# ZechengLi19/CIM

Hardware: AMD Instinct MI355X
Metric: images/sec training step (ResNet-50 VOC, ~1k proposals/img) at 1/2/4/8 GPU (higher is better)
Workload: dtype fp32

## Files before the change

### cim_amd/_lib.py

```python
import ctypes
import os

from ctypes import c_float, c_int, c_longlong, c_void_p

HERE = os.path.dirname(os.path.abspath(__file__))
LIB_PATH = os.environ.get("CIM_HIP_LIB") or os.path.join(HERE, "libcim_hip.so")

_P = c_void_p
SIGNATURES = {
    "cim_roi_align_fwd": [_P, _P, _P] + [c_int] * 6 + [c_float, c_int, c_int, _P],
    "cim_roi_align_fwd_ws": [_P, _P, _P] + [c_int] * 6 + [c_float, c_int, c_int, _P, _P],
    "cim_roi_align_maskcat_fwd_ws": [_P, _P, _P, _P] + [c_int] * 6 + [c_float, c_int, c_int, _P, _P],
    "cim_roi_align_wino7_pair_fwd": [_P, _P, _P, _P, _P] + [c_int] * 7 + [c_float, c_int, c_int, _P, _P],
    "cim_roi_align_bwd_ws": [_P, _P, _P] + [c_int] * 6 + [c_float, c_int, c_int, _P, c_int, _P, _P],
    "cim_roi_align_maskcat_bwd_ws": [_P, _P, _P, _P] + [c_int] * 6 + [c_float, c_int, c_int, _P, c_int, _P, _P],
    "cim_roi_align_bwd_workspace": [c_int, c_int, c_int, c_int],
    "cim_roi_align_bwd_scratch": [c_int, c_int, c_int, c_int, c_int],
    "cim_roi_align_bwd": [_P, _P, _P] + [c_int] * 6 + [c_float, c_int, c_int, _P, _P],
    "cim_roi_align_maskcat_fwd": [_P, _P, _P, _P] + [c_int] * 6 + [c_float, c_int, c_int, _P],
    "cim_roi_align_maskcat_bwd": [_P, _P, _P, _P] + [c_int] * 6 + [c_float, c_int, c_int, _P, _P],
    "cim_roi_align_forms": [c_int] * 9 + [_P] * 3,
    "cim_maxpool2d_out_size": [c_int, c_int, c_int, c_int],
    "cim_maxpool2d_fwd": [_P, _P, _P, c_int, c_int, c_int, c_int, c_int, c_int, _P],
    "cim_maxpool2d_bwd": [_P, _P, _P, c_int, c_int, c_int, c_int, c_int, c_int, _P],
    "cim_upsample_nearest_fwd": [_P, _P, c_int, c_int, c_int, c_int, c_int, _P],
    "cim_upsample_nearest_bwd": [_P, _P, c_int, c_int, c_int, c_int, _P],
    "cim_image_prep": [_P, c_int, c_int, _P, c_int, c_int, c_longlong, c_int, ctypes.c_double, c_int, _P, _P],
    "cim_mask_pack": [_P, _P, c_int, c_int, _P],
    "cim_mask_iou_pair": [_P, c_int, c_int, _P, _P, _P, _P],
    "cim_asy_flag": [_P, c_int, c_float, _P, _P],
    "cim_asy_prep": [_P, c_int, _P, c_int, _P, _P, _P],
    "cim_mining_step": [_P, _P, _P],
    "cim_mining_lds_bytes": [c_int, c_int],
    "cim_mining_sync_bytes": [],
    "cim_gemm_small_splits": [c_int, c_int, c_int],
    "cim_gemm_small_f32": [_P, _P, _P] + [c_int] * 8 + [_P, _P, _P, _P, _P, c_float, _P, c_int, c_int, _P, _P],
    "cim_conv1x1_bwd_workspace": [c_int, c_int, c_int, c_int],
    "cim_conv1x1_bn_act_bwd": [_P] * 8 + [c_float, c_int] + [_P] * 5 + [c_int] * 4 + [_P, _P, _P, _P, _P, c_int] + [c_int, _P, _P, c_float] + [_P] * 4 + [c_int],
    "cim_bn_part_finish": [_P, c_int, _P],
    "cim_conv3x3_nchw_splits": [c_int] * 5,
    "cim_conv3x3_nchw_f32": [_P, _P, _P] + [c_int] * 6 + [_P, _P, _P, _P, _P, c_float, _P, c_int, c_int, _P, _P],
    "cim_conv7x7_nchw_f32": [_P, _P, _P] + [c_int] * 5 + [_P, _P, _P, _P, c_float, c_int, _P],
    "cim_conv3x3_nchw_bwd_workspace": [c_int] * 6,
    "cim_conv3x3_dx_parts": [c_int] * 3,
    "cim_conv3x3_nchw_bn_act_bwd": [_P] * 8 + [c_float, c_int] + [_P] * 5 + [c_int] * 7 + [_P, _P, _P, _P, _P, c_int] + [c_int, _P, _P, c_float] + [_P] * 4,
    "cim_conv3x3_wt_multi": [_P, c_int, _P],
    "cim_bn_act_fwd": [_P, _P, _P, _P, _P, _P, c_float, _P, c_int, c_int, c_int, c_int, _P],
    "cim_bn_act_bwd_chunks": [c_int, c_int, c_int],
    "cim_bn_act_bwd": [_P, _P, _P, _P, _P, _P, c_float, _P, _P, _P, _P, c_int, c_int, c_int, c_int, _P],
    "cim_sgd_multi": [_P, _P, c_int, c_float, c_int, _P],
    "cim_gemm_pair_splits": [c_int, c_int, c_int],
    "cim_gemm_pair": [_P, _P, _P, _P] + [c_int] * 6 + [c_int, c_int, c_int, c_int, _P, _P, _P, _P, c_int, c_int, c_int, _P],
    "cim_gemm_pair_batched": [_P, _P, _P] + [c_int] * 6 + [c_int, c_int, c_int, c_longlong, c_longlong, c_longlong,
                              _P, _P, c_int, c_int, c_int, _P],
    "cim_pair_scales": [_P, c_int, _P, _P, c_int, c_int, _P],
    "cim_pair_split": [_P, _P, c_int, c_int, c_int, c_int, c_int, c_int, c_longlong, c_longlong, _P, _P, _P],
    "cim_pair_amax": [_P, c_longlong, _P, _P],
    "cim_pair_masked_stats": [_P, _P, c_int, c_int, _P, _P, _P],
# ... 57 lines not shown
    lib.cim_last_error.restype = ctypes.c_char_p
    lib.cim_last_error.argtypes = []
    lib.cim_abi_version.restype = c_int
    if lib.cim_abi_version() != ABI_VERSION:
        raise CimHipError("%s exports ABI %d, this package binds ABI %d: rebuild with `python -m cim_amd.build`"
                          % (LIB_PATH, lib.cim_abi_version(), ABI_VERSION))
    for name, argtypes in SIGNATURES.items():
        fn = getattr(lib, name)
        fn.argtypes = argtypes
        fn.restype = c_longlong if name in ("cim_conv1x1_bwd_workspace", "cim_conv3x3_nchw_bwd_workspace", "cim_roi_align_bwd_workspace", "cim_roi_align_bwd_scratch", "cim_mining_lds_bytes", "cim_mining_sync_bytes", "cim_detect_ws_bytes") or name in _LONG_RETURNING else c_int
    _lib = lib
    return lib


_LONG_RETURNING = {"cim_segm_rle_decode_ws_bytes", "cim_segm_image_ws_bytes", "cim_segm_record_bytes", "cim_segm_accumulate_ws_bytes", "cim_prop_ws_bytes"}
VALUE_RETURNING = _LONG_RETURNING | {"cim_segm_words"} | {"cim_maxpool2d_out_size", "cim_conv3x3_dx_parts", "cim_mining_sync_bytes", "cim_conv1x1_bwd_workspace", "cim_conv3x3_nchw_bwd_workspace", "cim_conv3x3_nchw_splits", "cim_gemm_small_splits", "cim_mining_lds_bytes", "cim_bn_act_bwd_chunks", "cim_gemm_pair_splits", "cim_roi_align_bwd_workspace", "cim_roi_align_bwd_scratch", "cim_detect_ws_bytes"}


PURE = {"cim_maxpool2d_out_size", "cim_conv3x3_dx_parts", "cim_gemm_small_splits", "cim_conv3x3_nchw_splits", "cim_conv1x1_bwd_workspace", "cim_conv3x3_nchw_bwd_workspace",
        "cim_bn_act_bwd_chunks", "cim_gemm_pair_splits"}
_PURE_VALUES = {}


def call(name, *args):
    if name in PURE:
        key = (name,) + args
        v = _PURE_VALUES.get(key)
        if v is None:
            v = _PURE_VALUES[key] = getattr(load(), name)(*args)
        return v
    lib = load()
    rc = getattr(lib, name)(*args)
    if name in VALUE_RETURNING:
        return rc
# ... 15 lines not shown
```

### cim_amd/csrc/conv1x1.hip

```cpp
#include "common.h"
#include "../../include/cim_hip.h"

#ifndef CIM_BODY_PRIO_LEVEL
#define CIM_BODY_PRIO_LEVEL 3
#endif
#if CIM_BODY_PRIO_LEVEL > 0
#define CIM_BODY_PRIO() __builtin_amdgcn_s_setprio(CIM_BODY_PRIO_LEVEL)
#else
#define CIM_BODY_PRIO()
#endif
namespace {

#ifndef CIM_SMALL_BK
#define CIM_SMALL_BK 32
#endif
#ifndef CIM_SMALL_ABL
#define CIM_SMALL_ABL 0
#endif
constexpr int SBM = 64, SBN = 64, SBK = CIM_SMALL_BK;
constexpr int SLD = 68;
typedef float f32x16 __attribute__((ext_vector_type(16)));
typedef float f32x4u __attribute__((ext_vector_type(4), aligned(4)));
__device__ __forceinline__ float4 ld4(const float* p) {
    const f32x4u v = *reinterpret_cast<const f32x4u*>(p);
    return make_float4(v.x, v.y, v.z, v.w);
}

struct SmallArgs {
    const float* A; const float* B; float* C; float* Xraw;
    const float* gamma; const float* beta; const float* mean; const float* var; const float* res;
    float eps;
    int M, N, K, lda, ldb, ldc;
    int a_mcontig, b_kcontig, relu, bn;
    int splits; float* ws;
    const float* colbias;
    const float* mask; const float* mgamma; const float* mvar; float meps;
    const float* mxr; const float* mmean; float* mpart; int mparts;
    int res_w, res_ws, res_hw;
};
struct InputBn { const float* y; const float* gamma; const float* var; float eps;
                 const float* xr; const float* mean; float* part; };

typedef unsigned int u32x4 __attribute__((ext_vector_type(4)));
typedef __amdgpu_buffer_rsrc_t rsrc_t;
__device__ __forceinline__ rsrc_t make_rsrc(const float* p, long long floats) {
    return __builtin_amdgcn_make_buffer_rsrc(const_cast<float*>(p), 0, (int)(unsigned)(floats * 4), 0x00020000);
}
__device__ __forceinline__ float4 bld4(rsrc_t r, unsigned byte_off) {
    const u32x4 v = __builtin_amdgcn_raw_buffer_load_b128(r, byte_off, 0, 0);
// ... 85 lines not shown
    __device__ __forceinline__ bool in(int c) const { return c < N; }
    __device__ __forceinline__ int col(int c) const { return c; }
    __device__ __forceinline__ int group(int c0) const { return c0 >> 5; }
};
struct ColParity {
    static constexpr bool splitk = false;
    int Wc, W, py, px, Nc, group0;
    __device__ __forceinline__ bool in(int c) const { return c < Nc; }
    __device__ __forceinline__ int col(int c) const {
        const int yc = c / Wc, xc = c - yc * Wc;
        return (2 * yc + py) * W + 2 * xc + px;
    }
    __device__ __forceinline__ int group(int c0) const { return group0 + (c0 >> 5); }
};
template <class Map>
__device__ __forceinline__ void small_epilogue(const SmallArgs& g, const f32x16& acc, int row0, int col0, int lane, int split, const Map& cm) {
#if CIM_SMALL_ABL == 2
    if (row0 + lane >= 0) return;
#endif
    const int nc = col0 + (lane & 31);
    if (Map::splitk && g.splits > 1) {
        if (cm.in(nc)) {
#pragma unroll
            for (int r = 0; r < 16; ++r) {
                const int row = row0 + 8 * (r >> 2) + 4 * (lane >> 5) + (r & 3);
                if (row < g.M) g.ws[((size_t)split * g.M + row) * g.N + cm.col(nc)] = acc[r];
            }
        }
        return;
    }
    const int col = cm.col(nc);
    if (g.mpart == nullptr) {
        if (cm.in(nc)) {
#pragma unroll
            for (int r = 0; r < 16; ++r) {
                const int row = row0 + 8 * (r >> 2) + 4 * (lane >> 5) + (r & 3);
                if (row < g.M) small_finish(g, row, col, acc[r]);
            }
        }
        return;
    }
#pragma unroll
    for (int r = 0; r < 16; ++r) {
        const int row = row0 + 8 * (r >> 2) + 4 * (lane >> 5) + (r & 3);
        float s1 = 0.0f, s2 = 0.0f;
        if (cm.in(nc) && row < g.M) small_finish(g, row, col, acc[r], s1, s2);
        small_put_part(g, row, cm.group(col0), lane, s1, s2);
    }
}


template <bool AM, bool BKc, int WN>
__global__ __launch_bounds__(128 * WN) void gemm_small_kernel(const SmallArgs g) {
    CIM_BODY_PRIO();
    constexpr int NT = 128 * WN, BNT = 32 * WN;
    constexpr int PA = SBM * 8 / NT, PB = BNT * 8 / NT;
    __shared__ __attribute__((aligned(16))) float As[2][SBK * SLD];
    __shared__ __attribute__((aligned(16))) float Bs[2][SBK * SLD];
    const int tid = threadIdx.x, lane = tid & 63, wave = tid >> 6;
    const int wm = wave / WN, wn = wave % WN;
    const int tiles_n = (g.N + BNT - 1) / BNT;
    const int tile = blockIdx.x;
    const int m0 = (tile / tiles_n) * SBM, n0 = (tile % tiles_n) * BNT;
    const int split = blockIdx.y;
    const int kper = ((g.K + g.splits - 1) / g.splits + SBK - 1) / SBK * SBK;
    const int kbeg = split * kper, kend = min(g.K, kbeg + kper);
#if CIM_SMALL_ABL == 4
    if (g.M > 0) return;
// ... 53 lines not shown
            SM_GLOAD(ra0, rb0, min(s + 2, last))
            SM_MMA(0)
            if (s + 1 < nslab) SM_PUT(ra1, rb1, 1, s + 1)
            __syncthreads();
            if (s + 1 >= nslab) break;
            SM_GLOAD(ra1, rb1, min(s + 3, last))
            SM_MMA(1)
            if (s + 2 < nslab) SM_PUT(ra0, rb0, 0, s + 2)
            __syncthreads();
        }
    }
#undef SM_GLOAD
#undef SM_PUT
#undef SM_MMA

    small_epilogue(g, acc, m0 + wm * 32, n0 + wn * 32, lane, split, ColIdentity{g.N});
}

__device__ __forceinline__ float splitk_sum(const float* __restrict__ ws, size_t i, size_t mn, int splits) {
    float v = ws[i];
    for (int k0 = 1; k0 < splits; k0 += 8) {
        float p[8];
#pragma unroll
        for (int j = 0; j < 8; ++j) p[j] = k0 + j < splits ? ws[(size_t)(k0 + j) * mn + i] : 0.0f;
#pragma unroll
        for (int j = 0; j < 8; ++j)
            if (k0 + j < splits) v += p[j];
    }
    return v;
}
__global__ __launch_bounds__(256) void small_splitk_reduce_kernel(const SmallArgs g) {
// ... 76 lines not shown
#pragma unroll
        for (int k = 0; k < 8; ++k) { a1 += sh[0][k][threadIdx.x]; a2 += sh[1][k][threadIdx.x]; }
        if (d.dbeta) d.dbeta[c] = a1;
        if (d.dgamma) d.dgamma[c] = a2 * rsqrtf(d.var[c] + d.eps);
    }
}

enum { CONV_FWD = 0, CONV_DX = 1, CONV_DW = 2 };
struct ConvGeom { int H, W, Ho, Wo, stride, cin, cout; float inv_w; int dil; };

#ifndef CIM_CONV3_BK
#define CIM_CONV3_BK 32
#endif
constexpr int CBK = CIM_CONV3_BK;
template <int MODE, int KS = 3>
__global__ __launch_bounds__(256) void conv3x3_small_kernel(const SmallArgs g, const ConvGeom c) {
    CIM_BODY_PRIO();
    constexpr int TAPS = KS * KS;
    constexpr int NT = 256, PA = SBM * (CBK / 4) / NT, PB = SBN * (CBK / 4) / NT;
    extern __shared__ __attribute__((aligned(16))) float c3_smem[];
    float (*As)[CBK * SLD] = reinterpret_cast<float (*)[CBK * SLD]>(c3_smem);
    float (*Bs)[CBK * SLD] = reinterpret_cast<float (*)[CBK * SLD]>(c3_smem + 2 * CBK * SLD);
    const int tid = threadIdx.x, lane = tid & 63, wave = tid >> 6;
    const int wm = wave >> 1, wn = wave & 1;
    const int tiles_n = (g.N + SBN - 1) / SBN;
    const int m0 = (blockIdx.x / tiles_n) * SBM, n0 = (blockIdx.x % tiles_n) * SBN;
    const int split = blockIdx.y;
    const int kper = ((g.K + g.splits - 1) / g.splits + CBK - 1) / CBK * CBK;
    const int kbeg = split * kper, kend = min(g.K, kbeg + kper);

    const rsrc_t RA_ = make_rsrc(g.A, tile_extent(MODE == CONV_DX, g.M, g.K, g.lda));
// ... 106 lines not shown
        __syncthreads();
        for (int s = 0; s < nslab; s += 2) {
            load_a(min(s + 2, last), ra0); load_b(kbeg + min(s + 2, last) * CBK, rb0);
            C3_MMA(0)
            if (s + 1 < nslab) C3_PUT(ra1, rb1, 1, s + 1)
            __syncthreads();
            if (s + 1 >= nslab) break;
            load_a(min(s + 3, last), ra1); load_b(kbeg + min(s + 3, last) * CBK, rb1);
            C3_MMA(1)
            if (s + 2 < nslab) C3_PUT(ra0, rb0, 0, s + 2)
            __syncthreads();
        }
    }
#undef C3_PUT
#undef C3_MMA
    small_epilogue(g, acc, m0 + wm * 32, n0 + wn * 32, lane, split, ColIdentity{g.N});
}

struct Dx2Geom { int H, W, Ho, Wo, cin, cout; int first[5]; int tiles_n[4]; int group0[4]; };

__global__ __launch_bounds__(256) void conv3x3_dx2_kernel(const SmallArgs g, const Dx2Geom c) {
    CIM_BODY_PRIO();
    constexpr int NT = 256, PA = SBM * (CBK / 4) / NT, PB = SBN * (CBK / 4) / NT;
    extern __shared__ __attribute__((aligned(16))) float d2_smem[];
    float (*As)[CBK * SLD] = reinterpret_cast<float (*)[CBK * SLD]>(d2_smem);
    float (*Bs)[CBK * SLD] = reinterpret_cast<float (*)[CBK * SLD]>(d2_smem + 2 * CBK * SLD);
    const int tid = threadIdx.x, lane = tid & 63, wave = tid >> 6;
    const int wm = wave >> 1, wn = wave & 1;
    int cls = 0;
    while (cls < 3 && (int)blockIdx.x >= c.first[cls + 1]) ++cls;
    const int py = cls >> 1, px = cls & 1;
// ... 174 lines not shown

extern "C" int cim_gemm_small_splits(int M, int N, int K) {
    const long long tiles = (long long)((M + SBM - 1) / SBM) * ((N + SBN - 1) / SBN);
#ifndef CIM_SMALL_WGS
#define CIM_SMALL_WGS 512
#endif
#ifndef CIM_SMALL_MINSLABS
#define CIM_SMALL_MINSLABS 4
#endif
    constexpr int min_k = CIM_SMALL_MINSLABS * SBK, want = CIM_SMALL_WGS;
    int s = 1;
    while (tiles * s < want && K / (s * 2) >= min_k && s < 64) s *= 2;
    return s;
}

static int gemm_small_impl(const float* A, const float* B, float* C, int M, int N, int K, int lda, int ldb, int ldc,
                           int a_mcontig, int b_kcontig, float* x_raw, const float* gamma, const float* beta,
                           const float* mean, const float* var, float eps, const float* residual, int relu, int splits,
                           float* workspace, void* stream, const InputBn* in_bn, int res_w = 0) {
    CIM_CHECK_ARG(res_w == 0 || (residual && res_w > 0 && N % res_w == 0 && ldc == N));
    CIM_CHECK_ARG(A && B && C && M > 0 && N > 0 && K > 0 && lda > 0 && ldb > 0 && ldc >= N && splits >= 1);
    CIM_CHECK_ARG((gamma == nullptr) == (beta == nullptr) && (gamma == nullptr) == (mean == nullptr) && (gamma == nullptr) == (var == nullptr));
    CIM_CHECK_ARG(splits == 1 || workspace);
    SmallArgs g = small_args(A, B, C, M, N, K, lda, ldb, ldc, splits, workspace, in_bn, x_raw, gamma, beta, mean, var, eps, residual, relu);
    g.a_mcontig = a_mcontig; g.b_kcontig = b_kcontig;
    g.res_w = res_w;
    if (res_w) { g.res_ws = (res_w + 1) / 2; g.res_hw = ((N / res_w + 1) / 2) * g.res_ws; }
    const long long tiles = (long long)((M + SBM - 1) / SBM) * ((N + SBN - 1) / SBN);
    CIM_CHECK_ARG(tiles * 2 < (1ll << 31) && splits <= 65535 && M <= 65535);
    CIM_CHECK_ARG(tile_extent(a_mcontig != 0, M, K, lda) < (1ll << 29) && tile_extent(b_kcontig == 0, N, K, ldb) < (1ll << 29));
    const bool narrow = tiles * splits < 128;
    hipStream_t st = cim::as_stream(stream);
    if (a_mcontig) {
        if (b_kcontig) launch_small<true, true>(g, splits, st, narrow); else launch_small<true, false>(g, splits, st, narrow);
    } else {
        if (b_kcontig) launch_small<false, true>(g, splits, st, narrow); else launch_small<false, false>(g, splits, st, narrow);
    }
    if (splits > 1) launch_splitk_reduce(g, st);
    CIM_CHECK_LAUNCH();
    return 0;
}

extern "C" int cim_gemm_small_f32(const float* A, const float* B, float* C, int M, int N, int K, int lda, int ldb, int ldc,
                                  int a_mcontig, int b_kcontig, float* x_raw, const float* gamma, const float* beta,
                                  const float* mean, const float* var, float eps, const float* residual, int relu, int splits,
                                  float* workspace, void* stream) {
    return gemm_small_impl(A, B, C, M, N, K, lda, ldb, ldc, a_mcontig, b_kcontig, x_raw, gamma, beta, mean, var, eps, residual, relu,
                           splits, workspace, stream, nullptr);
}

extern "C" int cim_linear_bias_f32(const float* X, const float* W, const float* bias, float* Y, int M, int N, int K, int splits,
                                   float* workspace, void* stream) {
    CIM_CHECK_ARG(X && W && Y && M > 0 && N > 0 && K > 0 && splits >= 1 && splits <= 65535 && (splits == 1 || workspace));
    SmallArgs g = small_args(X, W, Y, M, N, K, K, K, N, splits, workspace, nullptr);
    g.b_kcontig = 1; g.colbias = bias;
// ... 39 lines not shown
    const size_t i = (size_t)blockIdx.x * 256 + threadIdx.x;
    if (i < n) y[i] += x[i];
}
template <class Product>
int dw_over_images(int B, float* dw, float* ws_dw, int sp, size_t n, hipStream_t st, Product product) {
    for (int b = 0; b < B && dw; ++b) {
        float* out = b == 0 ? dw : ws_dw + (size_t)sp * n;
        const int rc = product(b, out);
        if (rc) return rc;
        if (b) hipLaunchKernelGGL(small_axpy_kernel, dim3((unsigned)((n + 255) / 256)), dim3(256), 0, st, dw, out, n);
    }
    return 0;
}
}

extern "C" int cim_conv1x1_bn_act_bwd(const float* dy, const float* y, const float* x_raw, const float* x, const float* w,
                                      const float* gamma, const float* mean, const float* var, float eps, int relu,
                                      float* dres, float* dgamma, float* dbeta, float* dx, float* dw, int B, int cin, int cout,
                                      int hw, float* workspace, void* stream, void* side_stream, void* fork_event, void* join_event, int join,
                                      int dy_is_dconv, const float* in_gamma, const float* in_var, float in_eps,
                                      const float* in_xr, const float* in_mean, float* in_part, const float* dx_add, int dx_add_w) {
    CIM_CHECK_ARG(dx_add_w == 0 || (dx_add != nullptr && dx_add_w > 0 && hw % dx_add_w == 0));
    CIM_CHECK_ARG(side_stream == nullptr || side_stream == stream || (fork_event != nullptr && (!join || join_event != nullptr)));
    const size_t add_bs = dx_add_w ? (size_t)cin * ((hw / dx_add_w + 1) / 2) * ((dx_add_w + 1) / 2) : (size_t)cin * hw;
    CIM_CHECK_ARG(dy && x_raw && x && w && gamma && mean && var && workspace && B > 0 && cin > 0 && cout > 0 && hw > 0);
    CIM_CHECK_ARG(dx_add == nullptr || (dx != nullptr && in_gamma == nullptr));
    CIM_CHECK_ARG((y != nullptr || !relu) && ((dgamma == nullptr) == (dbeta == nullptr)));
    CIM_CHECK_ARG(!dy_is_dconv || (dres == nullptr && dgamma == nullptr));
    CIM_CHECK_ARG((in_gamma == nullptr) == (in_var == nullptr));
    CIM_CHECK_ARG(in_part == nullptr || (in_gamma && in_xr && in_mean));
    float* dconv = dy_is_dconv ? const_cast<float*>(dy) : workspace;
    float* ws_dx = workspace + (size_t)B * cout * hw;
    float* ws_dw = ws_dx + (size_t)cim_gemm_small_splits(cin, hw, cout) * cin * hw;
    int rc = dy_is_dconv ? 0 : cim_bn_act_bwd(dy, y, x_raw, gamma, mean, var, eps, dconv, dres, dgamma, dbeta, B, cout, hw, relu, stream);
    if (rc) return rc;
    ForkJoin fj(cim::as_stream(stream), cim::as_stream(side_stream), fork_event, join_event, dx && dw);
    hipStream_t st_dw = fj.fork();
    const int sp = cim_gemm_small_splits(cout, cin, hw);
    rc = dw_over_images(B, dw, ws_dw, sp, (size_t)cout * cin, st_dw, [&](int b, float* out) {
        return cim_gemm_small_f32(dconv + (size_t)b * cout * hw, x + (size_t)b * cin * hw, out, cout, cin, hw, hw, hw, cin, 0, 1,
                                  nullptr, nullptr, nullptr, nullptr, nullptr, 0.f, nullptr, 0, sp, ws_dw, st_dw);
    });
    if (rc) return rc;
    for (int b = 0; b < B && dx; ++b) {
        const InputBn ib{x + (size_t)b * cin * hw, in_gamma, in_var, in_eps, in_xr ? in_xr + (size_t)b * cin * hw : nullptr, in_mean,
                         in_part ? in_part + (size_t)b * 2 * ((hw + 31) / 32) * cin : nullptr};
        rc = gemm_small_impl(w, dconv + (size_t)b * cout * hw, dx + (size_t)b * cin * hw, cin, hw, cout, cin, hw, hw, 1, 0,
                             nullptr, nullptr, nullptr, nullptr, nullptr, 0.f, dx_add ? dx_add + (size_t)b * add_bs : nullptr, 0,
                             cim_gemm_small_splits(cin, hw, cout), ws_dx, stream, in_gamma ? &ib : nullptr, dx_add_w);
        if (rc) return rc;
    }
    if (join) fj.join();
    CIM_CHECK_LAUNCH();
    return 0;
}

namespace {
int conv3x3_launch(int mode, const float* A, const float* B, float* C, int M, int N, int K, int lda, int ldc, const ConvGeom& c,
                   float* x_raw, const float* gamma, const float* beta, const float* mean, const float* var, float eps,
                   const float* residual, int relu, int splits, float* ws, hipStream_t st, int ksize = 3, const InputBn* in_bn = nullptr) {
    SmallArgs g = small_args(A, B, C, M, N, K, lda, 0, ldc, splits, ws, in_bn, x_raw, gamma, beta, mean, var, eps, residual, relu);
    g.b_kcontig = mode == CONV_DW;
    const dim3 grid((unsigned)(((M + SBM - 1) / SBM) * ((N + SBN - 1) / SBN)), (unsigned)splits);
    auto kern = ksize == 7 ? conv3x3_small_kernel<CONV_FWD, 7>
                : mode == CONV_FWD ? conv3x3_small_kernel<CONV_FWD> : mode == CONV_DX ? conv3x3_small_kernel<CONV_DX> : conv3x3_small_kernel<CONV_DW>;
    const int rc = launch_lds(kern, grid, sizeof(float) * 4 * CBK * SLD, st, g, c);
    if (rc) return rc;
    if (splits > 1) launch_splitk_reduce(g, st);
    return 0;
}
ConvGeom conv_geom(int cin, int cout, int H, int W, int stride, int mode, int dil = 1) {
    ConvGeom c;
    c.H = H; c.W = W; c.stride = stride; c.cin = cin; c.cout = cout; c.dil = dil;
    c.Ho = (H - 1) / stride + 1; c.Wo = (W - 1) / stride + 1;
    c.inv_w = 1.0f / (float)(mode == CONV_DX ? W : c.Wo);
    return c;
}
}

#define CONV3_ARGS_OK(CIN_MULT)                                                                                      \
    CIM_CHECK_ARG(cin > 0 && cout > 0 && H > 0 && W > 0 && (stride == 1 || stride == 2) && W <= 4096 &&               \
                  dilation >= 1 && dilation <= 8 && (dilation == 1 || stride == 1) &&                                 \
                  (long long)H * W < (1ll << 20) && (long long)cin * H * W < (1ll << 29) && (long long)cout * H * W < (1ll << 29) && \
                  (long long)cin * cout * 9 < (1ll << 29) && cin % (CIN_MULT) == 0)

extern "C" int cim_conv3x3_nchw_splits(int cin, int cout, int H, int W, int stride) {
    const int Ho = (H - 1) / stride + 1, Wo = (W - 1) / stride + 1;
    return cim_gemm_small_splits(cout, Ho * Wo, 9 * cin);
}

extern "C" int cim_conv3x3_nchw_f32(const float* x, const float* w, float* y, int cin, int cout, int H, int W, int stride,
                               int dilation, float* x_raw, const float* gamma, const float* beta, const float* mean, const float* var,
                               float eps, const float* residual, int relu, int splits, float* workspace, void* stream) {
    CIM_CHECK_ARG(x && w && y && splits >= 1 && splits <= 65535 && (splits == 1 || workspace));
    CONV3_ARGS_OK(1);
    CIM_CHECK_ARG((gamma == nullptr) == (beta == nullptr) && (gamma == nullptr) == (mean == nullptr) && (gamma == nullptr) == (var == nullptr));
    const ConvGeom c = conv_geom(cin, cout, H, W, stride, CONV_FWD, dilation);
    conv3x3_launch(CONV_FWD, w, x, y, cout, c.Ho * c.Wo, 9 * cin, 9 * cin, c.Ho * c.Wo, c, x_raw, gamma, beta, mean, var, eps,
                   residual, relu, splits, workspace, cim::as_stream(stream));
    CIM_CHECK_LAUNCH();
    return 0;
}

extern "C" int cim_conv7x7_nchw_f32(const float* x, const float* w, float* y, int cin, int cout, int H, int W, int stride,
                                    const float* gamma, const float* beta, const float* mean, const float* var, float eps,
                                    int relu, void* stream) {
    CIM_CHECK_ARG(x && w && y && cin > 0 && cout > 0 && H > 0 && W > 0 && (stride == 1 || stride == 2) && W <= 4096);
    CIM_CHECK_ARG((long long)H * W < (1ll << 20) && (long long)cin * H * W < (1ll << 29) && (long long)cout * H * W < (1ll << 29));
    CIM_CHECK_ARG((gamma == nullptr) == (beta == nullptr) && (gamma == nullptr) == (mean == nullptr) && (gamma == nullptr) == (var == nullptr));
    const ConvGeom c = conv_geom(cin, cout, H, W, stride, CONV_FWD);
    conv3x3_launch(CONV_FWD, w, x, y, cout, c.Ho * c.Wo, 49 * cin, 49 * cin, c.Ho * c.Wo, c, nullptr, gamma, beta, mean, var, eps,
                   nullptr, relu, 1, nullptr, cim::as_stream(stream), 7);
    CIM_CHECK_LAUNCH();
    return 0;
}

// ... 64 lines not shown
            const cim_wt_desc& d = descs[base + i];
            CIM_CHECK_ARG(d.w && d.wt && d.cin > 0 && d.cout > 0 && (size_t)d.cin * 9 * sizeof(float) <= 64 * 1024);
            t.d[i] = d;
            t.first[i] = total;
            total += d.cout;
            max_cin = d.cin > max_cin ? d.cin : max_cin;
        }
        t.first[t.n] = total;
        const int rc = launch_lds(conv3x3_wt_multi_kernel, dim3((unsigned)total), sizeof(float) * max_cin * 9, st, t);
        if (rc) return rc;
    }
    CIM_CHECK_LAUNCH();
    return 0;
}

extern "C" int cim_conv3x3_nchw_bn_act_bwd(const float* dy, const float* y, const float* x_raw, const float* x, const float* w,
                                      const float* gamma, const float* mean, const float* var, float eps, int relu,
                                      float* dres, float* dgamma, float* dbeta, float* dx, float* dw, int B, int cin, int cout,
                                      int H, int W, int stride, int dilation, float* workspace, void* stream, void* side_stream,
                                      void* fork_event, void* join_event, int join, int dy_is_dconv, const float* in_gamma, const float* in_var, float in_eps,
                                      const float* in_xr, const float* in_mean, float* in_part, const float* wt_ready) {
    CIM_CHECK_ARG(dy && x_raw && x && w && gamma && mean && var && workspace && B > 0);
    CIM_CHECK_ARG(side_stream == nullptr || side_stream == stream || (fork_event != nullptr && (!join || join_event != nullptr)));
    CONV3_ARGS_OK(4);
    CIM_CHECK_ARG((y != nullptr || !relu) && ((dgamma == nullptr) == (dbeta == nullptr)) && cout % 4 == 0);
    CIM_CHECK_ARG(!dy_is_dconv || (dres == nullptr && dgamma == nullptr));
    CIM_CHECK_ARG((in_gamma == nullptr) == (in_var == nullptr));
    CIM_CHECK_ARG(in_part == nullptr || (in_gamma && in_xr && in_mean));
    const ConvGeom cx = conv_geom(cin, cout, H, W, stride, CONV_DX, dilation), cw = conv_geom(cin, cout, H, W, stride, CONV_DW, dilation);
    const int hwo = cx.Ho * cx.Wo, hw = H * W;
    hipStream_t st = cim::as_stream(stream);
    float* dconv = dy_is_dconv ? const_cast<float*>(dy) : workspace;
    float* wt_own = workspace + (size_t)B * cout * hwo;
    const float* wt = wt_ready ? wt_ready : wt_own;
    float* ws_dx = wt_own + (size_t)cout * cin * 9;
    float* ws_dw = ws_dx + (size_t)cim_gemm_small_splits(cin, hw, 9 * cout) * cin * hw;
// ... 12 lines not shown
    const int parts = cim_conv3x3_dx_parts(H, W, dilation == 1 ? stride : 1);
    for (int b = 0; b < B && dx; ++b) {
        const InputBn ib{x + (size_t)b * cin * hw, in_gamma, in_var, in_eps, in_xr ? in_xr + (size_t)b * cin * hw : nullptr, in_mean,
                         in_part ? in_part + (size_t)b * 2 * parts * cin : nullptr};
        if (stride == 2 && dilation == 1) {
            SmallArgs g = small_args(wt, dconv + (size_t)b * cout * hwo, dx + (size_t)b * cin * hw, cin, hw, 9 * cout, cin, 0, hw, 1, nullptr,
                                     in_gamma ? &ib : nullptr);
            g.mparts = parts;
            const Dx2Geom c2 = dx2_geom(cin, cout, H, W);
            rc = launch_lds(conv3x3_dx2_kernel, dim3((unsigned)c2.first[4]), sizeof(float) * 4 * CBK * SLD, st, g, c2);
            if (rc) return rc;
            continue;
        }
        conv3x3_launch(CONV_DX, wt, dconv + (size_t)b * cout * hwo, dx + (size_t)b * cin * hw, cin, hw, 9 * cout, cin, hw, cx, nullptr,
                       nullptr, nullptr, nullptr, nullptr, 0.f, nullptr, 0, cim_gemm_small_splits(cin, hw, 9 * cout), ws_dx, st, 3,
                       in_gamma ? &ib : nullptr);
    }
    if (join) fj.join();
    CIM_CHECK_LAUNCH();
    return 0;
}
```

### include/cim_hip.h

```cpp
#ifndef CIM_HIP_H
#define CIM_HIP_H

#include <stdint.h>

#ifdef __cplusplus
extern "C" {
#endif

const char* cim_last_error(void);
int cim_abi_version(void);

int cim_roi_align_fwd(const float* feat, const float* rois, float* out,
                      int B, int C, int H, int W, int K, int P,
                      float spatial_scale, int sampling_ratio, int aligned, void* stream);

long long cim_roi_align_bwd_workspace(int K, int P, int H, int W);
int cim_roi_align_bwd(const float* grad_out, const float* rois, float* grad_in,
                      int B, int C, int H, int W, int K, int P,
                      float spatial_scale, int sampling_ratio, int aligned, float* workspace, void* stream);

int cim_roi_align_fwd_ws(const float* feat, const float* rois, float* out,
                         int B, int C, int H, int W, int K, int P,
                         float spatial_scale, int sampling_ratio, int aligned, float* workspace, void* stream);
int cim_roi_align_maskcat_fwd_ws(const float* feat, const float* rois, const float* masks, float* cat,
// ... 118 lines not shown

int cim_image_prep(const uint8_t* src_bgr, int h, int w, float* dst, int H, int W, long long plane_stride, int row_stride,
                   double inv_scale, int hflip, const float* mean_std6_host, void* stream);

int cim_maxpool2d_out_size(int in, int k, int stride, int pad);
int cim_maxpool2d_fwd(const float* x, float* y, int* idx, int NC, int H, int W, int k, int stride, int pad, void* stream);
int cim_maxpool2d_bwd(const float* dy, const int* idx, float* dx, int NC, int H, int W, int k, int stride, int pad, void* stream);
int cim_upsample_nearest_fwd(const float* x, float* y, int NC, int H, int W, int scale, int accumulate, void* stream);
int cim_upsample_nearest_bwd(const float* dy, float* dx, int NC, int H, int W, int scale, void* stream);

int cim_gemm_small_splits(int M, int N, int K);
int cim_gemm_small_f32(const float* A, const float* B, float* C, int M, int N, int K, int lda, int ldb, int ldc,
                       int a_mcontig, int b_kcontig, float* x_raw, const float* gamma, const float* beta,
                       const float* mean, const float* var, float eps, const float* residual, int relu, int splits,
                       float* workspace, void* stream);

long long cim_conv1x1_bwd_workspace(int B, int cin, int cout, int hw);
int cim_conv1x1_bn_act_bwd(const float* dy, const float* y, const float* x_raw, const float* x, const float* w,
                           const float* gamma, const float* mean, const float* var, float eps, int relu,
                           float* dres, float* dgamma, float* dbeta, float* dx, float* dw, int B, int cin, int cout, int hw,
                           float* workspace, void* stream, void* side_stream, void* fork_event, void* join_event, int join,
                           int dy_is_dconv, const float* in_gamma, const float* in_var, float in_eps,
                           const float* in_xr, const float* in_mean, float* in_part, const float* dx_add, int dx_add_w);
typedef struct { const float* part; const float* var; float eps; float* dgamma; float* dbeta; int images; int parts; int channels; } cim_bn_part_desc;
int cim_bn_part_finish(const cim_bn_part_desc* descs, int n, void* stream);

int cim_conv3x3_nchw_splits(int cin, int cout, int H, int W, int stride);
int cim_conv3x3_nchw_f32(const float* x, const float* w, float* y, int cin, int cout, int H, int W, int stride, int dilation,
                         float* x_raw, const float* gamma, const float* beta, const float* mean, const float* var, float eps,
                         const float* residual, int relu, int splits, float* workspace, void* stream);
int cim_conv7x7_nchw_f32(const float* x, const float* w, float* y, int cin, int cout, int H, int W, int stride,
                         const float* gamma, const float* beta, const float* mean, const float* var, float eps, int relu,
                         void* stream);
long long cim_conv3x3_nchw_bwd_workspace(int B, int cin, int cout, int H, int W, int stride);
int cim_conv3x3_dx_parts(int H, int W, int stride);
int cim_conv3x3_nchw_bn_act_bwd(const float* dy, const float* y, const float* x_raw, const float* x, const float* w,
                                const float* gamma, const float* mean, const float* var, float eps, int relu, float* dres,
                                float* dgamma, float* dbeta, float* dx, float* dw, int B, int cin, int cout, int H, int W,
                                int stride, int dilation, float* workspace, void* stream, void* side_stream, void* fork_event,
                                void* join_event, int join, int dy_is_dconv, const float* in_gamma, const float* in_var, float in_eps,
                                const float* in_xr, const float* in_mean, float* in_part, const float* wt_ready);
typedef struct { const float* w; float* wt; int cin; int cout; } cim_wt_desc;
int cim_conv3x3_wt_multi(const cim_wt_desc* descs, int n, void* stream);

int cim_bn_act_fwd(const float* x, const float* res, const float* gamma, const float* beta, const float* mean,
                   const float* var, float eps, float* y, int N, int C, int HW, int relu, void* stream);
int cim_bn_act_bwd_chunks(int N, int C, int HW);
int cim_bn_act_bwd(const float* dy, const float* y, const float* x, const float* gamma, const float* mean,
                   const float* var, float eps, float* dx, float* dres, float* dgamma, float* dbeta,
                   int N, int C, int HW, int relu, void* stream);

int cim_gemm_pair_splits(int M, int N, int K);
int cim_gemm_pair(const void* A, const void* B, float* C, const float* bias, int M, int N, int K,
                  int lda, int ldb, int ldc, int a_mcontig, int b_kcontig, int relu, int splits, float* workspace,
                  const float* a_scale, const float* b_scale, uint32_t* c_amax, int max_workgroups, int products, int form,
                  void* stream);
// ... 79 lines not shown
```

Baseline: 77.08.

## Fold split-K reduction into last-arriving workgroup via atomic tickets

New measurement: 76.05. 0.987x the previous value.

```diff
diff --git a/cim_amd/_lib.py b/cim_amd/_lib.py
--- a/cim_amd/_lib.py
+++ b/cim_amd/_lib.py
@@ -35,13 +35,19 @@
     "cim_mining_sync_bytes": [],
     "cim_gemm_small_splits": [c_int, c_int, c_int],
     "cim_gemm_small_f32": [_P, _P, _P] + [c_int] * 8 + [_P, _P, _P, _P, _P, c_float, _P, c_int, c_int, _P, _P],
+    "cim_splitk_ticket_words": [],
+    "cim_gemm_small_fold": [c_int, c_int, c_int, c_int],
+    "cim_gemm_small_fold_f32": [_P, _P, _P] + [c_int] * 8 + [_P, _P, _P, _P, _P, c_float, _P, c_int, c_int, _P, _P, _P],
     "cim_conv1x1_bwd_workspace": [c_int, c_int, c_int, c_int],
+    "cim_conv1x1_bn_act_bwd_fold": [_P] * 8 + [c_float, c_int] + [_P] * 5 + [c_int] * 4 + [_P, _P, _P, _P, _P, c_int] + [c_int, _P, _P, c_float] + [_P] * 4 + [c_int, _P],
     "cim_conv1x1_bn_act_bwd": [_P] * 8 + [c_float, c_int] + [_P] * 5 + [c_int] * 4 + [_P, _P, _P, _P, _P, c_int] + [c_int, _P, _P, c_float] + [_P] * 4 + [c_int],
     "cim_bn_part_finish": [_P, c_int, _P],
     "cim_conv3x3_nchw_splits": [c_int] * 5,
     "cim_conv3x3_nchw_f32": [_P, _P, _P] + [c_int] * 6 + [_P, _P, _P, _P, _P, c_float, _P, c_int, c_int, _P, _P],
     "cim_conv7x7_nchw_f32": [_P, _P, _P] + [c_int] * 5 + [_P, _P, _P, _P, c_float, c_int, _P],
+    "cim_conv3x3_nchw_fold_f32": [_P, _P, _P] + [c_int] * 6 + [_P, _P, _P, _P, _P, c_float, _P, c_int, c_int, _P, _P, _P],
     "cim_conv3x3_nchw_bwd_workspace": [c_int] * 6,
+    "cim_conv3x3_nchw_bn_act_bwd_fold": [_P] * 8 + [c_float, c_int] + [_P] * 5 + [c_int] * 7 + [_P, _P, _P, _P, _P, c_int] + [c_int, _P, _P, c_float] + [_P] * 4 + [_P],
     "cim_conv3x3_dx_parts": [c_int] * 3,
     "cim_conv3x3_nchw_bn_act_bwd": [_P] * 8 + [c_float, c_int] + [_P] * 5 + [c_int] * 7 + [_P, _P, _P, _P, _P, c_int] + [c_int, _P, _P, c_float] + [_P] * 4,
     "cim_conv3x3_wt_multi": [_P, c_int, _P],
@@ -129,10 +135,10 @@
 
 
 _LONG_RETURNING = {"cim_segm_rle_decode_ws_bytes", "cim_segm_image_ws_bytes", "cim_segm_record_bytes", "cim_segm_accumulate_ws_bytes", "cim_prop_ws_bytes"}
-VALUE_RETURNING = _LONG_RETURNING | {"cim_segm_words"} | {"cim_maxpool2d_out_size", "cim_conv3x3_dx_parts", "cim_mining_sync_bytes", "cim_conv1x1_bwd_workspace", "cim_conv3x3_nchw_bwd_workspace", "cim_conv3x3_nchw_splits", "cim_gemm_small_splits", "cim_mining_lds_bytes", "cim_bn_act_bwd_chunks", "cim_gemm_pair_splits", "cim_roi_align_bwd_workspace", "cim_roi_align_bwd_scratch", "cim_detect_ws_bytes"}
+VALUE_RETURNING = _LONG_RETURNING | {"cim_segm_words", "cim_splitk_ticket_words", "cim_gemm_small_fold"} | {"cim_maxpool2d_out_size", "cim_conv3x3_dx_parts", "cim_mining_sync_bytes", "cim_conv1x1_bwd_workspace", "cim_conv3x3_nchw_bwd_workspace", "cim_conv3x3_nchw_splits", "cim_gemm_small_splits", "cim_mining_lds_bytes", "cim_bn_act_bwd_chunks", "cim_gemm_pair_splits", "cim_roi_align_bwd_workspace", "cim_roi_align_bwd_scratch", "cim_detect_ws_bytes"}
 
 
-PURE = {"cim_maxpool2d_out_size", "cim_conv3x3_dx_parts", "cim_gemm_small_splits", "cim_conv3x3_nchw_splits", "cim_conv1x1_bwd_workspace", "cim_conv3x3_nchw_bwd_workspace",
+PURE = {"cim_splitk_ticket_words", "cim_gemm_small_fold", "cim_maxpool2d_out_size", "cim_conv3x3_dx_parts", "cim_gemm_small_splits", "cim_conv3x3_nchw_splits", "cim_conv1x1_bwd_workspace", "cim_conv3x3_nchw_bwd_workspace",
         "cim_bn_act_bwd_chunks", "cim_gemm_pair_splits"}
 _PURE_VALUES = {}
 
diff --git a/cim_amd/csrc/conv1x1.hip b/cim_amd/csrc/conv1x1.hip
--- a/cim_amd/csrc/conv1x1.hip
+++ b/cim_amd/csrc/conv1x1.hip
@@ -33,6 +33,7 @@
     int M, N, K, lda, ldb, ldc;
     int a_mcontig, b_kcontig, relu, bn;
     int splits; float* ws;
+    unsigned* tickets;
     const float* colbias;
     const float* mask; const float* mgamma; const float* mvar; float meps;
     const float* mxr; const float* mmean; float* mpart; int mparts;
@@ -148,21 +149,8 @@
     __device__ __forceinline__ int group(int c0) const { return group0 + (c0 >> 5); }
 };
 template <class Map>
-__device__ __forceinline__ void small_epilogue(const SmallArgs& g, const f32x16& acc, int row0, int col0, int lane, int split, const Map& cm) {
-#if CIM_SMALL_ABL == 2
-    if (row0 + lane >= 0) return;
-#endif
+__device__ __forceinline__ void small_tile_finish(const SmallArgs& g, const f32x16& acc, int row0, int col0, int lane, const Map& cm) {
     const int nc = col0 + (lane & 31);
-    if (Map::splitk && g.splits > 1) {
-        if (cm.in(nc)) {
-#pragma unroll
-            for (int r = 0; r < 16; ++r) {
-                const int row = row0 + 8 * (r >> 2) + 4 * (lane >> 5) + (r & 3);
-                if (row < g.M) g.ws[((size_t)split * g.M + row) * g.N + cm.col(nc)] = acc[r];
-            }
-        }
-        return;
-    }
     const int col = cm.col(nc);
     if (g.mpart == nullptr) {
         if (cm.in(nc)) {
@@ -182,10 +170,70 @@
         small_put_part(g, row, cm.group(col0), lane, s1, s2);
     }
 }
+template <class Map>
+__device__ __forceinline__ void small_epilogue(const SmallArgs& g, const f32x16& acc, int row0, int col0, int lane, int split, const Map& cm,
+                                               int tile = 0, int* flag = nullptr) {
+#if CIM_SMALL_ABL == 2
+    if (row0 + lane >= 0) return;
+#endif
+    if (!(Map::splitk && g.splits > 1)) {
+        small_tile_finish(g, acc, row0, col0, lane, cm);
+        return;
+    }
+    const int nc = col0 + (lane & 31);
+    if (g.tickets == nullptr) {
+        if (cm.in(nc)) {
+#pragma unroll
+            for (int r = 0; r < 16; ++r) {
+                const int row = row0 + 8 * (r >> 2) + 4 * (lane >> 5) + (r & 3);
+                if (row < g.M) g.ws[((size_t)split * g.M + row) * g.N + cm.col(nc)] = acc[r];
+            }
+        }
+        return;
+    }
+    if (cm.in(nc)) {
+#pragma unroll
+        for (int r = 0; r < 16; ++r) {
+            const int row = row0 + 8 * (r >> 2) + 4 * (lane >> 5) + (r & 3);
+            if (row < g.M) __hip_atomic_store(g.ws + ((size_t)split * g.M + row) * g.N + cm.col(nc), acc[r], __ATOMIC_RELAXED, __HIP_MEMORY_SCOPE_AGENT);
+        }
+    }
+    asm volatile("s_waitcnt vmcnt(0)" ::: "memory");
+    __syncthreads();
+    if (threadIdx.x == 0) {
+        const unsigned t = __hip_atomic_fetch_add(g.tickets + tile, 1u, __ATOMIC_RELAXED, __HIP_MEMORY_SCOPE_AGENT);
+        const int last = t == (unsigned)g.splits - 1u;
+        if (last) {
+            __hip_atomic_store(g.tickets + tile, 0u, __ATOMIC_RELAXED, __HIP_MEMORY_SCOPE_AGENT);
+            __builtin_amdgcn_fence(__ATOMIC_ACQUIRE, "agent");
+            asm volatile("s_waitcnt vmcnt(0)" ::: "memory");
+        }
+        *flag = last;
+    }
+    __syncthreads();
+    if (*flag == 0) return;
+    const unsigned mn = (unsigned)g.M * (unsigned)g.N;
+    const unsigned lc = (unsigned)min(cm.col(nc), g.N - 1);
+    const int rl = row0 + 4 * (lane >> 5);
+    f32x16 v;
+#pragma unroll
+    for (int r = 0; r < 16; ++r)
+        v[r] = __hip_atomic_load(g.ws + ((unsigned)min(rl + 8 * (r >> 2) + (r & 3), g.M - 1) * (unsigned)g.N + lc), __ATOMIC_RELAXED, __HIP_MEMORY_SCOPE_AGENT);
+    for (int k = 1; k < g.splits; ++k) {
+        const float* __restrict__ p = g.ws + (size_t)k * mn;
+        float a[16];
+#pragma unroll
+        for (int r = 0; r < 16; ++r)
+            a[r] = __hip_atomic_load(p + ((unsigned)min(rl + 8 * (r >> 2) + (r & 3), g.M - 1) * (unsigned)g.N + lc), __ATOMIC_RELAXED, __HIP_MEMORY_SCOPE_AGENT);
+#pragma unroll
+        for (int r = 0; r < 16; ++r) v[r] += a[r];
+    }
+    small_tile_finish(g, v, row0, col0, lane, cm);
+}
 
 
 template <bool AM, bool BKc, int WN>
-__global__ __launch_bounds__(128 * WN) void gemm_small_kernel(const SmallArgs g) {
+__global__ __launch_bounds__(128 * WN) __attribute__((amdgpu_num_vgpr(96))) void gemm_small_kernel(const SmallArgs g) {
     CIM_BODY_PRIO();
     constexpr int NT = 128 * WN, BNT = 32 * WN;
     constexpr int PA = SBM * 8 / NT, PB = BNT * 8 / NT;
@@ -269,7 +317,7 @@
 #undef SM_PUT
 #undef SM_MMA
 
-    small_epilogue(g, acc, m0 + wm * 32, n0 + wn * 32, lane, split, ColIdentity{g.N});
+    small_epilogue(g, acc, m0 + wm * 32, n0 + wn * 32, lane, split, ColIdentity{g.N}, tile, reinterpret_cast<int*>(&As[0][0]));
 }
 
 __device__ __forceinline__ float splitk_sum(const float* __restrict__ ws, size_t i, size_t mn, int splits) {
@@ -376,7 +424,7 @@
 #endif
 constexpr int CBK = CIM_CONV3_BK;
 template <int MODE, int KS = 3>
-__global__ __launch_bounds__(256) void conv3x3_small_kernel(const SmallArgs g, const ConvGeom c) {
+__global__ __launch_bounds__(256) __attribute__((amdgpu_num_vgpr(96))) void conv3x3_small_kernel(const SmallArgs g, const ConvGeom c) {
     CIM_BODY_PRIO();
     constexpr int TAPS = KS * KS;
     constexpr int NT = 256, PA = SBM * (CBK / 4) / NT, PB = SBN * (CBK / 4) / NT;
@@ -513,7 +561,7 @@
     }
 #undef C3_PUT
 #undef C3_MMA
-    small_epilogue(g, acc, m0 + wm * 32, n0 + wn * 32, lane, split, ColIdentity{g.N});
+    small_epilogue(g, acc, m0 + wm * 32, n0 + wn * 32, lane, split, ColIdentity{g.N}, (int)blockIdx.x, reinterpret_cast<int*>(c3_smem));
 }
 
 struct Dx2Geom { int H, W, Ho, Wo, cin, cout; int first[5]; int tiles_n[4]; int group0[4]; };
@@ -718,16 +766,35 @@
     return s;
 }
 
+#ifndef CIM_SMALL_FOLD
+#define CIM_SMALL_FOLD 1
+#endif
+#ifndef CIM_SMALL_FOLD_MAX
+#define CIM_SMALL_FOLD_MAX 8
+#endif
+constexpr int SMALL_TICKETS = 1024;
+extern "C" int cim_splitk_ticket_words(void) { return SMALL_TICKETS; }
+static bool small_fold(long long launched_tiles, int splits, long long mn) {
+    return CIM_SMALL_FOLD && splits > 1 && splits <= CIM_SMALL_FOLD_MAX && launched_tiles <= SMALL_TICKETS && mn < (1ll << 31);
+}
+extern "C" int cim_gemm_small_fold(int M, int N, int K, int splits) {
+    (void)K;
+    const long long tm = (M + SBM - 1) / SBM;
+    const long long tiles = tm * ((N + SBN - 1) / SBN);
+    return small_fold(tiles * splits < 128 ? tm * ((N + 31) / 32) : tiles, splits, (long long)M * N);
+}
+
 static int gemm_small_impl(const float* A, const float* B, float* C, int M, int N, int K, int lda, int ldb, int ldc,
                            int a_mcontig, int b_kcontig, float* x_raw, const float* gamma, const float* beta,
                            const float* mean, const float* var, float eps, const float* residual, int relu, int splits,
-                           float* workspace, void* stream, const InputBn* in_bn, int res_w = 0) {
+                           float* workspace, void* stream, const InputBn* in_bn, int res_w = 0, unsigned* tickets = nullptr) {
     CIM_CHECK_ARG(res_w == 0 || (residual && res_w > 0 && N % res_w == 0 && ldc == N));
     CIM_CHECK_ARG(A && B && C && M > 0 && N > 0 && K > 0 && lda > 0 && ldb > 0 && ldc >= N && splits >= 1);
     CIM_CHECK_ARG((gamma == nullptr) == (beta == nullptr) && (gamma == nullptr) == (mean == nullptr) && (gamma == nullptr) == (var == nullptr));
     CIM_CHECK_ARG(splits == 1 || workspace);
     SmallArgs g = small_args(A, B, C, M, N, K, lda, ldb, ldc, splits, workspace, in_bn, x_raw, gamma, beta, mean, var, eps, residual, relu);
     g.a_mcontig = a_mcontig; g.b_kcontig = b_kcontig;
+    g.tickets = tickets && cim_gemm_small_fold(M, N, K, splits) ? tickets : nullptr;
     g.res_w = res_w;
     if (res_w) { g.res_ws = (res_w + 1) / 2; g.res_hw = ((N / res_w + 1) / 2) * g.res_ws; }
     const long long tiles = (long long)((M + SBM - 1) / SBM) * ((N + SBN - 1) / SBN);
@@ -740,9 +807,17 @@
     } else {
         if (b_kcontig) launch_small<false, true>(g, splits, st, narrow); else launch_small<false, false>(g, splits, st, narrow);
     }
-    if (splits > 1) launch_splitk_reduce(g, st);
+    if (splits > 1 && !g.tickets) launch_splitk_reduce(g, st);
     CIM_CHECK_LAUNCH();
     return 0;
+}
+
+extern "C" int cim_gemm_small_fold_f32(const float* A, const float* B, float* C, int M, int N, int K, int lda, int ldb, int ldc,
+                                       int a_mcontig, int b_kcontig, float* x_raw, const float* gamma, const float* beta,
+                                       const float* mean, const float* var, float eps, const float* residual, int relu, int splits,
+                                       float* workspace, void* stream, unsigned* tickets) {
+    return gemm_small_impl(A, B, C, M, N, K, lda, ldb, ldc, a_mcontig, b_kcontig, x_raw, gamma, beta, mean, var, eps, residual, relu,
+                           splits, workspace, stream, nullptr, 0, tickets);
 }
 
 extern "C" int cim_gemm_small_f32(const float* A, const float* B, float* C, int M, int N, int K, int lda, int ldb, int ldc,
@@ -812,12 +887,13 @@
 }
 }
 
-extern "C" int cim_conv1x1_bn_act_bwd(const float* dy, const float* y, const float* x_raw, const float* x, const float* w,
+static int conv1x1_bwd_impl(const float* dy, const float* y, const float* x_raw, const float* x, const float* w,
                                       const float* gamma, const float* mean, const float* var, float eps, int relu,
                                       float* dres, float* dgamma, float* dbeta, float* dx, float* dw, int B, int cin, int cout,
                                       int hw, float* workspace, void* stream, void* side_stream, void* fork_event, void* join_event, int join,
                                       int dy_is_dconv, const float* in_gamma, const float* in_var, float in_eps,
-                                      const float* in_xr, const float* in_mean, float* in_part, const float* dx_add, int dx_add_w) {
+                                      const float* in_xr, const float* in_mean, float* in_part, const float* dx_add, int dx_add_w,
+                                      unsigned* tickets) {
     CIM_CHECK_ARG(dx_add_w == 0 || (dx_add != nullptr && dx_add_w > 0 && hw % dx_add_w == 0));
     CIM_CHECK_ARG(side_stream == nullptr || side_stream == stream || (fork_event != nullptr && (!join || join_event != nullptr)));
     const size_t add_bs = dx_add_w ? (size_t)cin * ((hw / dx_add_w + 1) / 2) * ((dx_add_w + 1) / 2) : (size_t)cin * hw;
@@ -845,26 +921,49 @@
                          in_part ? in_part + (size_t)b * 2 * ((hw + 31) / 32) * cin : nullptr};
         rc = gemm_small_impl(w, dconv + (size_t)b * cout * hw, dx + (size_t)b * cin * hw, cin, hw, cout, cin, hw, hw, 1, 0,
                              nullptr, nullptr, nullptr, nullptr, nullptr, 0.f, dx_add ? dx_add + (size_t)b * add_bs : nullptr, 0,
-                             cim_gemm_small_splits(cin, hw, cout), ws_dx, stream, in_gamma ? &ib : nullptr, dx_add_w);
+                             cim_gemm_small_splits(cin, hw, cout), ws_dx, stream, in_gamma ? &ib : nullptr, dx_add_w, tickets);
         if (rc) return rc;
     }
     if (join) fj.join();
     CIM_CHECK_LAUNCH();
     return 0;
 }
+extern "C" int cim_conv1x1_bn_act_bwd(const float* dy, const float* y, const float* x_raw, const float* x, const float* w,
+                                      const float* gamma, const float* mean, const float* var, float eps, int relu,
+                                      float* dres, float* dgamma, float* dbeta, float* dx, float* dw, int B, int cin, int cout,
+                                      int hw, float* workspace, void* stream, void* side_stream, void* fork_event, void* join_event, int join,
+                                      int dy_is_dconv, const float* in_gamma, const float* in_var, float in_eps,
+                                      const float* in_xr, const float* in_mean, float* in_part, const float* dx_add, int dx_add_w) {
+    return conv1x1_bwd_impl(dy, y, x_raw, x, w, gamma, mean, var, eps, relu, dres, dgamma, dbeta, dx, dw, B, cin, cout, hw, workspace, stream,
+                            side_stream, fork_event, join_event, join, dy_is_dconv, in_gamma, in_var, in_eps, in_xr, in_mean, in_part, dx_add,
+                            dx_add_w, nullptr);
+}
+extern "C" int cim_conv1x1_bn_act_bwd_fold(const float* dy, const float* y, const float* x_raw, const float* x, const float* w,
+                                      const float* gamma, const float* mean, const float* var, float eps, int relu,
+                                      float* dres, float* dgamma, float* dbeta, float* dx, float* dw, int B, int cin, int cout,
+                                      int hw, float* workspace, void* stream, void* side_stream, void* fork_event, void* join_event, int join,
+                                      int dy_is_dconv, const float* in_gamma, const float* in_var, float in_eps,
+                                      const float* in_xr, const float* in_mean, float* in_part, const float* dx_add, int dx_add_w,
+                                      unsigned* tickets) {
+    return conv1x1_bwd_impl(dy, y, x_raw, x, w, gamma, mean, var, eps, relu, dres, dgamma, dbeta, dx, dw, B, cin, cout, hw, workspace, stream,
+                            side_stream, fork_event, join_event, join, dy_is_dconv, in_gamma, in_var, in_eps, in_xr, in_mean, in_part, dx_add,
+                            dx_add_w, tickets);
+}
 
 namespace {
 int conv3x3_launch(int mode, const float* A, const float* B, float* C, int M, int N, int K, int lda, int ldc, const ConvGeom& c,
                    float* x_raw, const float* gamma, const float* beta, const float* mean, const float* var, float eps,
-                   const float* residual, int relu, int splits, float* ws, hipStream_t st, int ksize = 3, const InputBn* in_bn = nullptr) {
+                   const float* residual, int relu, int splits, float* ws, hipStream_t st, int ksize = 3, const InputBn* in_bn = nullptr,
+                   unsigned* tickets = nullptr) {
     SmallArgs g = small_args(A, B, C, M, N, K, lda, 0, ldc, splits, ws, in_bn, x_raw, gamma, beta, mean, var, eps, residual, relu);
     g.b_kcontig = mode == CONV_DW;
     const dim3 grid((unsigned)(((M + SBM - 1) / SBM) * ((N + SBN - 1) / SBN)), (unsigned)splits);
+    g.tickets = tickets && small_fold(grid.x, splits, (long long)M * N) ? tickets : nullptr;
     auto kern = ksize == 7 ? conv3x3_small_kernel<CONV_FWD, 7>
                 : mode == CONV_FWD ? conv3x3_small_kernel<CONV_FWD> : mode == CONV_DX ? conv3x3_small_kernel<CONV_DX> : conv3x3_small_kernel<CONV_DW>;
     const int rc = launch_lds(kern, grid, sizeof(float) * 4 * CBK * SLD, st, g, c);
     if (rc) return rc;
-    if (splits > 1) launch_splitk_reduce(g, st);
+    if (splits > 1 && !g.tickets) launch_splitk_reduce(g, st);
     return 0;
 }
 ConvGeom conv_geom(int cin, int cout, int H, int W, int stride, int mode, int dil = 1) {
@@ -887,17 +986,29 @@
     return cim_gemm_small_splits(cout, Ho * Wo, 9 * cin);
 }
 
-extern "C" int cim_conv3x3_nchw_f32(const float* x, const float* w, float* y, int cin, int cout, int H, int W, int stride,
+static int conv3x3_fwd_impl(const float* x, const float* w, float* y, int cin, int cout, int H, int W, int stride,
                                int dilation, float* x_raw, const float* gamma, const float* beta, const float* mean, const float* var,
-                               float eps, const float* residual, int relu, int splits, float* workspace, void* stream) {
+                               float eps, const float* residual, int relu, int splits, float* workspace, void* stream, unsigned* tickets) {
     CIM_CHECK_ARG(x && w && y && splits >= 1 && splits <= 65535 && (splits == 1 || workspace));
     CONV3_ARGS_OK(1);
     CIM_CHECK_ARG((gamma == nullptr) == (beta == nullptr) && (gamma == nullptr) == (mean == nullptr) && (gamma == nullptr) == (var == nullptr));
     const ConvGeom c = conv_geom(cin, cout, H, W, stride, CONV_FWD, dilation);
     conv3x3_launch(CONV_FWD, w, x, y, cout, c.Ho * c.Wo, 9 * cin, 9 * cin, c.Ho * c.Wo, c, x_raw, gamma, beta, mean, var, eps,
-                   residual, relu, splits, workspace, cim::as_stream(stream));
+                   residual, relu, splits, workspace, cim::as_stream(stream), 3, nullptr, tickets);
     CIM_CHECK_LAUNCH();
     return 0;
+}
+extern "C" int cim_conv3x3_nchw_f32(const float* x, const float* w, float* y, int cin, int cout, int H, int W, int stride,
+                               int dilation, float* x_raw, const float* gamma, const float* beta, const float* mean, const float* var,
+                               float eps, const float* residual, int relu, int splits, float* workspace, void* stream) {
+    return conv3x3_fwd_impl(x, w, y, cin, cout, H, W, stride, dilation, x_raw, gamma, beta, mean, var, eps, residual, relu, splits, workspace,
+                            stream, nullptr);
+}
+extern "C" int cim_conv3x3_nchw_fold_f32(const float* x, const float* w, float* y, int cin, int cout, int H, int W, int stride,
+                               int dilation, float* x_raw, const float* gamma, const float* beta, const float* mean, const float* var,
+                               float eps, const float* residual, int relu, int splits, float* workspace, void* stream, unsigned* tickets) {
+    return conv3x3_fwd_impl(x, w, y, cin, cout, H, W, stride, dilation, x_raw, gamma, beta, mean, var, eps, residual, relu, splits, workspace,
+                            stream, tickets);
 }
 
 extern "C" int cim_conv7x7_nchw_f32(const float* x, const float* w, float* y, int cin, int cout, int H, int W, int stride,
@@ -992,12 +1103,12 @@
     return 0;
 }
 
-extern "C" int cim_conv3x3_nchw_bn_act_bwd(const float* dy, const float* y, const float* x_raw, const float* x, const float* w,
+static int conv3x3_bwd_impl(const float* dy, const float* y, const float* x_raw, const float* x, const float* w,
                                       const float* gamma, const float* mean, const float* var, float eps, int relu,
                                       float* dres, float* dgamma, float* dbeta, float* dx, float* dw, int B, int cin, int cout,
                                       int H, int W, int stride, int dilation, float* workspace, void* stream, void* side_stream,
                                       void* fork_event, void* join_event, int join, int dy_is_dconv, const float* in_gamma, const float* in_var, float in_eps,
-                                      const float* in_xr, const float* in_mean, float* in_part, const float* wt_ready) {
+                                      const float* in_xr, const float* in_mean, float* in_part, const float* wt_ready, unsigned* tickets) {
     CIM_CHECK_ARG(dy && x_raw && x && w && gamma && mean && var && workspace && B > 0);
     CIM_CHECK_ARG(side_stream == nullptr || side_stream == stream || (fork_event != nullptr && (!join || join_event != nullptr)));
     CONV3_ARGS_OK(4);
@@ -1040,9 +1151,29 @@
         }
         conv3x3_launch(CONV_DX, wt, dconv + (size_t)b * cout * hwo, dx + (size_t)b * cin * hw, cin, hw, 9 * cout, cin, hw, cx, nullptr,
                        nullptr, nullptr, nullptr, nullptr, 0.f, nullptr, 0, cim_gemm_small_splits(cin, hw, 9 * cout), ws_dx, st, 3,
-                       in_gamma ? &ib : nullptr);
+                       in_gamma ? &ib : nullptr, tickets);
     }
     if (join) fj.join();
     CIM_CHECK_LAUNCH();
     return 0;
 }
+extern "C" int cim_conv3x3_nchw_bn_act_bwd(const float* dy, const float* y, const float* x_raw, const float* x, const float* w,
+                                      const float* gamma, const float* mean, const float* var, float eps, int relu,
+                                      float* dres, float* dgamma, float* dbeta, float* dx, float* dw, int B, int cin, int cout,
+                                      int H, int W, int stride, int dilation, float* workspace, void* stream, void* side_stream,
+                                      void* fork_event, void* join_event, int join, int dy_is_dconv, const float* in_gamma, const float* in_var, float in_eps,
+                                      const float* in_xr, const float* in_mean, float* in_part, const float* wt_ready) {
+    return conv3x3_bwd_impl(dy, y, x_raw, x, w, gamma, mean, var, eps, relu, dres, dgamma, dbeta, dx, dw, B, cin, cout, H, W, stride, dilation,
+                            workspace, stream, side_stream, fork_event, join_event, join, dy_is_dconv, in_gamma, in_var, in_eps, in_xr, in_mean,
+                            in_part, wt_ready, nullptr);
+}
+extern "C" int cim_conv3x3_nchw_bn_act_bwd_fold(const float* dy, const float* y, const float* x_raw, const float* x, const float* w,
+                                      const float* gamma, const float* mean, const float* var, float eps, int relu,
+                                      float* dres, float* dgamma, float* dbeta, float* dx, float* dw, int B, int cin, int cout,
+                                      int H, int W, int stride, int dilation, float* workspace, void* stream, void* side_stream,
+                                      void* fork_event, void* join_event, int join, int dy_is_dconv, const float* in_gamma, const float* in_var, float in_eps,
+                                      const float* in_xr, const float* in_mean, float* in_part, const float* wt_ready, unsigned* tickets) {
+    return conv3x3_bwd_impl(dy, y, x_raw, x, w, gamma, mean, var, eps, relu, dres, dgamma, dbeta, dx, dw, B, cin, cout, H, W, stride, dilation,
+                            workspace, stream, side_stream, fork_event, join_event, join, dy_is_dconv, in_gamma, in_var, in_eps, in_xr, in_mean,
+                            in_part, wt_ready, tickets);
+}
diff --git a/include/cim_hip.h b/include/cim_hip.h
--- a/include/cim_hip.h
+++ b/include/cim_hip.h
@@ -156,6 +156,12 @@
                        int a_mcontig, int b_kcontig, float* x_raw, const float* gamma, const float* beta,
                        const float* mean, const float* var, float eps, const float* residual, int relu, int splits,
                        float* workspace, void* stream);
+int cim_splitk_ticket_words(void);
+int cim_gemm_small_fold(int M, int N, int K, int splits);
+int cim_gemm_small_fold_f32(const float* A, const float* B, float* C, int M, int N, int K, int lda, int ldb, int ldc,
+                            int a_mcontig, int b_kcontig, float* x_raw, const float* gamma, const float* beta,
+                            const float* mean, const float* var, float eps, const float* residual, int relu, int splits,
+                            float* workspace, void* stream, unsigned* tickets);
 
 long long cim_conv1x1_bwd_workspace(int B, int cin, int cout, int hw);
 int cim_conv1x1_bn_act_bwd(const float* dy, const float* y, const float* x_raw, const float* x, const float* w,
@@ -164,6 +170,13 @@
                            float* workspace, void* stream, void* side_stream, void* fork_event, void* join_event, int join,
                            int dy_is_dconv, const float* in_gamma, const float* in_var, float in_eps,
                            const float* in_xr, const float* in_mean, float* in_part, const float* dx_add, int dx_add_w);
+int cim_conv1x1_bn_act_bwd_fold(const float* dy, const float* y, const float* x_raw, const float* x, const float* w,
+                           const float* gamma, const float* mean, const float* var, float eps, int relu,
+                           float* dres, float* dgamma, float* dbeta, float* dx, float* dw, int B, int cin, int cout, int hw,
+                           float* workspace, void* stream, void* side_stream, void* fork_event, void* join_event, int join,
+                           int dy_is_dconv, const float* in_gamma, const float* in_var, float in_eps,
+                           const float* in_xr, const float* in_mean, float* in_part, const float* dx_add, int dx_add_w,
+                           unsigned* tickets);
 typedef struct { const float* part; const float* var; float eps; float* dgamma; float* dbeta; int images; int parts; int channels; } cim_bn_part_desc;
 int cim_bn_part_finish(const cim_bn_part_desc* descs, int n, void* stream);
 
@@ -171,6 +184,9 @@
 int cim_conv3x3_nchw_f32(const float* x, const float* w, float* y, int cin, int cout, int H, int W, int stride, int dilation,
                          float* x_raw, const float* gamma, const float* beta, const float* mean, const float* var, float eps,
                          const float* residual, int relu, int splits, float* workspace, void* stream);
+int cim_conv3x3_nchw_fold_f32(const float* x, const float* w, float* y, int cin, int cout, int H, int W, int stride, int dilation,
+                         float* x_raw, const float* gamma, const float* beta, const float* mean, const float* var, float eps,
+                         const float* residual, int relu, int splits, float* workspace, void* stream, unsigned* tickets);
 int cim_conv7x7_nchw_f32(const float* x, const float* w, float* y, int cin, int cout, int H, int W, int stride,
                          const float* gamma, const float* beta, const float* mean, const float* var, float eps, int relu,
                          void* stream);
@@ -182,6 +198,12 @@
                                 int stride, int dilation, float* workspace, void* stream, void* side_stream, void* fork_event,
                                 void* join_event, int join, int dy_is_dconv, const float* in_gamma, const float* in_var, float in_eps,
                                 const float* in_xr, const float* in_mean, float* in_part, const float* wt_ready);
+int cim_conv3x3_nchw_bn_act_bwd_fold(const float* dy, const float* y, const float* x_raw, const float* x, const float* w,
+                                const float* gamma, const float* mean, const float* var, float eps, int relu, float* dres,
+                                float* dgamma, float* dbeta, float* dx, float* dw, int B, int cin, int cout, int H, int W,
+                                int stride, int dilation, float* workspace, void* stream, void* side_stream, void* fork_event,
+                                void* join_event, int join, int dy_is_dconv, const float* in_gamma, const float* in_var, float in_eps,
+                                const float* in_xr, const float* in_mean, float* in_part, const float* wt_ready, unsigned* tickets);
 typedef struct { const float* w; float* wt; int cin; int cout; } cim_wt_desc;
 int cim_conv3x3_wt_multi(const cim_wt_desc* descs, int n, void* stream);
 
```
